# JasonTStanley/MultiDroneSim

Hardware: AMD Instinct MI355X
Metric: drone-steps/sec (whole node) at N_envs×N_drones; achieved HBM GB/s vs roofline (higher is better)
Workload: dtype f32

## Files before the change

include/mds.h:

```cpp
#ifndef MDS_H
#define MDS_H

#include <stddef.h>
#include <stdint.h>

#ifdef __cplusplus
extern "C" {
#endif

#define MDS_VERSION 202
#define MDS_OBS_DIM 20
#define MDS_ACT_DIM 4
#define MDS_STATE_DIM 13
#define MDS_DES_DIM 11
#define MDS_LEM_DIM 7
#define MDS_GEO_AUX_DIM 13

typedef enum mds_status {
  MDS_OK = 0,
  MDS_EINVAL = -1,
  MDS_ENOMEM = -2,
  MDS_EHIP = -3,
  MDS_EALIGN = -4,
  MDS_ESTATE = -5,
// ... 55 lines not shown
int mds_step(mds_handle* h, const void* action_dev, void* obs_dev, void* stream);

int mds_set_wind(mds_handle* h, const double force_world[3]);

#define MDS_SEG_DIM 40
int mds_set_trajectory_segments(mds_handle* h, const double* segs_host, const int32_t* offsets_host,
                                const int32_t* compound_host, const double* anchor_host, int32_t total_segments, void* stream);
int mds_traj_eval(mds_handle* h, double t, void* des_dev, void* stream);

int mds_set_lemniscate(mds_handle* h, const double* params_host, void* stream);
int mds_traj_yaw_free(mds_handle* h);
int mds_set_traj_specialisation(mds_handle* h, int on);
int mds_traj_phase_periodic(mds_handle* h);
int mds_set_traj_phase_table(mds_handle* h, int on);
int mds_get_last_rollout_phase_table(mds_handle* h);
int mds_set_geometric_gains(mds_handle* h, const mds_geometric_gains* gains);

int mds_step_geometric(mds_handle* h, double t, void* obs_dev, void* action_dev, void* stream);

int mds_rollout_geometric(mds_handle* h, double t0, int n_steps, void* obs_dev, int obs_every_step, void* stream);

int mds_rollout_step(mds_handle* h, const void* actions_dev, int n_action_sets, int first_step, int n_steps, void* obs_log_dev,
                     int log_slots, int episode_len, void* stream);
int mds_rollout_step_fused(mds_handle* h, const void* actions_dev, int n_action_sets, int first_step, int n_steps, void* obs_log_dev,
                           int log_slots, int episode_len, int steps_per_launch, void* stream);
int mds_reset_async(mds_handle* h, void* stream);

typedef struct mds_episode_params {
  int32_t max_steps;
  int32_t reserved;
// ... 155 lines not shown
```

multidronesim_amd/_capi.py:

```python
from __future__ import annotations

import ctypes as C
import os

_HERE = os.path.dirname(os.path.abspath(__file__))
LIB_PATH = os.environ.get("MDS_LIB_PATH") or os.path.join(_HERE, "libmds.so")

MDS_OK = 0
MDS_F32, MDS_F64, MDS_F16, MDS_F32C = 0, 1, 2, 3
MDS_PHYSICS_DYN, MDS_PHYSICS_DYN_DRAG, MDS_PHYSICS_DYN_GND, MDS_PHYSICS_DYN_DW, MDS_PHYSICS_DYN_GND_DRAG_DW = 0, 1, 2, 3, 4
MDS_INTEGRATOR_EULER, MDS_INTEGRATOR_RK4 = 0, 1
MDS_CF2X, MDS_CF2P = 0, 1
OBS_DIM, ACT_DIM, STATE_DIM, DES_DIM, LEM_DIM, GEO_AUX_DIM, SEG_DIM = 20, 4, 13, 11, 7, 13, 40


class MdsConfig(C.Structure):
    _fields_ = [("num_envs", C.c_int32), ("num_drones", C.c_int32), ("dtype", C.c_int32), ("physics", C.c_int32),
                ("integrator", C.c_int32), ("drone_model", C.c_int32), ("pyb_freq", C.c_int32),
                ("ctrl_freq", C.c_int32), ("device", C.c_int32), ("track_last_rpm", C.c_int32),
                ("M", C.c_double), ("L", C.c_double), ("KF", C.c_double), ("KM", C.c_double), ("J", C.c_double * 3),
                ("G", C.c_double), ("thrust2weight", C.c_double), ("drag_coeff", C.c_double * 3)]


class MdsGeometricGains(C.Structure):
# ... 47 lines not shown
    "mds_get_derived": (C.c_int, [_P, _PD]),
    "mds_reset": (C.c_int, [_P, _PD, _PD, _P]),
    "mds_state_ptrs": (C.c_int, [_P, C.POINTER(C.c_void_p), C.POINTER(C.c_size_t), C.POINTER(C.c_void_p)]),
    "mds_get_state": (C.c_int, [_P, _PD, _P]),
    "mds_set_state": (C.c_int, [_P, _PD, _P]),
    "mds_set_origin": (C.c_int, [_P, _PD, _P]),
    "mds_get_obs": (C.c_int, [_P, _P, _P]),
    "mds_step": (C.c_int, [_P, _P, _P, _P]),
    "mds_set_wind": (C.c_int, [_P, _PD]),
    "mds_set_lemniscate": (C.c_int, [_P, _PD, _P]),
    "mds_traj_yaw_free": (C.c_int, [_P]),
    "mds_set_traj_specialisation": (C.c_int, [_P, C.c_int]),
    "mds_traj_phase_periodic": (C.c_int, [_P]),
    "mds_set_traj_phase_table": (C.c_int, [_P, C.c_int]),
    "mds_get_last_rollout_phase_table": (C.c_int, [_P]),
    "mds_set_trajectory_segments": (C.c_int, [_P, _PD, C.POINTER(C.c_int32), C.POINTER(C.c_int32), _PD, C.c_int32, _P]),
    "mds_traj_eval": (C.c_int, [_P, C.c_double, _P, _P]),
    "mds_set_geometric_gains": (C.c_int, [_P, C.POINTER(MdsGeometricGains)]),
    "mds_step_geometric": (C.c_int, [_P, C.c_double, _P, _P, _P]),
    "mds_rollout_geometric": (C.c_int, [_P, C.c_double, C.c_int, _P, C.c_int, _P]),
    "mds_set_rollout_streams": (C.c_int, [_P, C.c_int]),
    "mds_get_last_rollout_streams": (C.c_int, [_P]),
    "mds_rollout_streams_for": (C.c_int, [_P, C.c_int, C.c_int]),
    "mds_set_rollout_form": (C.c_int, [_P, C.c_int, C.c_int]),
    "mds_rollout_form_for": (C.c_int, [_P, C.c_int]),
    "mds_get_last_rollout_form": (C.c_int, [_P]),
    "mds_rollout_step": (C.c_int, [_P, _P, C.c_int, C.c_int, C.c_int, _P, C.c_int, C.c_int, _P]),
    "mds_rollout_step_fused": (C.c_int, [_P, _P, C.c_int, C.c_int, C.c_int, _P, C.c_int, C.c_int, C.c_int, _P]),
    "mds_reset_async": (C.c_int, [_P, _P]),
    "mds_default_episode_params": (C.c_int, [C.POINTER(MdsEpisodeParams)]),
# ... 120 lines not shown
```

multidronesim_amd/csrc/mds_api.hip:

```cpp
#include <hip/hip_runtime.h>
#include <math.h>
#include <stdio.h>
#include <stdlib.h>
#include <string.h>

#include <new>
#include <type_traits>
#include <unordered_map>
#include <vector>

#include "../../include/mds.h"
#include "mds_consts.hpp"
#include "mds_devmem.hpp"
#include "mds_kernels.hip"
#include "mds_traj_image.hpp"
#ifndef MDS_PART
#define MDS_PART 3
#endif
#if MDS_PART & 1
#include "mds_episode_kernels.hip"
#endif
#if MDS_PART & 2
#include "mds_cbf_kernels.hip"
#include "mds_fedce_kernels.hip"
// ... 99 lines not shown
  void* lem = nullptr;
  double* scratch = nullptr;
  double* init_pose = nullptr;
  bool has_traj = false;
  int traj_mode = 0;
  bool traj_yaw_free = false;
  bool traj_spec = true;
  bool traj_phase_periodic = false;
  bool phase_tab_on = true;
  void* phase_tab = nullptr;
  bool phase_tab_filled = false;
  int phase_tab_rows = 0;
  int phase_tab_row = 0;
  double phase_tab_t = 0.0;
  int last_rollout_phase_table = 0;
  double* segs = nullptr;
  int nseg_total = 0;
  int* tinfo = nullptr;
  HostParams<float> p32 = {};
  HostParams<double> p64 = {};
  bool has_cbf = false;
  mds_cbf_params cbf = {};
  int* pair_ij = nullptr;
  void* obstacles = nullptr;
  int* cbf_order = nullptr;
  int* cbf_count = nullptr;
  int cbf_calls_half[2] = {-1, -1};
  int* cbf_cost = nullptr;
  int cbf_calls = -1;
  int rollout_streams = 0;
// ... 626 lines not shown
  return envfx_return_home(h, home, st);
}

int mds_step(mds_handle* h, const void* action, void* obs, void* stream) {
  MDS_DEV(h);
  if (!h || !action) return fail(MDS_EINVAL, "mds_step: null argument");
  if (!aligned16(action) || !aligned16(obs)) return fail(MDS_EALIGN, "mds_step: action_dev/obs_dev");
  if (int rc = step_plain(h, action, obs, Chain{(hipStream_t)stream, 0, 0})) return rc;
  return check_launches();
}

constexpr int kPhaseTabRows = 2048;
static bool phase_table_built(const mds_handle* h) {
  return h->cfg.dtype == MDS_F32 && h->cfg.integrator != MDS_INTEGRATOR_RK4 && !has_drag(h) && !h->envfx;
}
static size_t phase_table_bytes(const mds_handle* h) { return (size_t)kPhaseTabRows * kPhaseLanes * 2 * comp_size(h->cfg.dtype); }

int mds_set_lemniscate(mds_handle* h, const double* params, void* stream) {
  MDS_DEV(h);
  if (!h || !params) return fail(MDS_EINVAL, "mds_set_lemniscate: null argument");
  hipStream_t st = (hipStream_t)stream;
  const int n = h->n;
  double* centres = new (std::nothrow) double[(size_t)n * 3];
  if (!centres) return fail(MDS_ENOMEM, "mds_set_lemniscate: host allocation");
  bool yaw_free = true;
  for (int i = 0; i < n; ++i) {
    for (int k = 0; k < 3; ++k) centres[(size_t)3 * i + k] = params[(size_t)7 * i + 2 + k];
    yaw_free = yaw_free && params[(size_t)7 * i + 5] == 0.0;
  }
  const bool phase_periodic = lemniscate_phase_periodic(params, n);
  if (yaw_free && phase_periodic && phase_table_built(h))
    if (int arc = h->mem.alloc(&h->phase_tab, phase_table_bytes(h))) {
      delete[] centres;
      return arc;
    }
  int rc = mds_set_origin(h, centres, stream);
  delete[] centres;
  if (rc != MDS_OK) return rc;
  MDS_HIP(hipMemcpyAsync(h->scratch, params, (size_t)n * 7 * sizeof(double), hipMemcpyHostToDevice, st));
  with_dtype(h->cfg.dtype, [&](auto DT) {
    using T = typename decltype(DT)::T;
    k_set_planes<T><<<grid_for(n, 256), 256, 0, st>>>(n, h->ld, 7, h->scratch, (T*)h->lem);
  });
  MDS_HIP(hipGetLastError());
  MDS_HIP(hipStreamSynchronize(st));
  h->has_traj = true;
  h->traj_mode = 1;
  h->traj_yaw_free = yaw_free;
  h->traj_phase_periodic = phase_periodic;
  h->phase_tab_filled = false;
  return MDS_OK;
}

int mds_traj_yaw_free(mds_handle* h) { return h && h->traj_yaw_free ? 1 : 0; }
int mds_traj_phase_periodic(mds_handle* h) { return h && h->traj_phase_periodic ? 1 : 0; }

int mds_set_traj_specialisation(mds_handle* h, int on) {
  if (!h) return fail(MDS_EINVAL, "mds_set_traj_specialisation: null handle");
  h->traj_spec = on != 0;
  return MDS_OK;
}

int mds_set_traj_phase_table(mds_handle* h, int on) {
  if (!h) return fail(MDS_EINVAL, "mds_set_traj_phase_table: null handle");
  h->phase_tab_on = on != 0;
  return MDS_OK;
}

int mds_get_last_rollout_phase_table(mds_handle* h) { return h ? h->last_rollout_phase_table : 0; }

static bool use_yaw_free(const mds_handle* h) { return h->traj_mode == 1 && h->traj_yaw_free && h->traj_spec; }

int mds_set_trajectory_segments(mds_handle* h, const double* segs, const int32_t* offsets, const int32_t* compound,
                                const double* anchor, int32_t total, void* stream) {
  MDS_DEV(h);
  if (!h || !segs || !offsets || !compound || !anchor) return fail(MDS_EINVAL, "mds_set_trajectory_segments: null argument");
  const int n = h->n;
  std::vector<int> ti;
  std::vector<double> fm;
  int nu = 0;
  const char* why = "";
  const int brc = build_traj_image(segs, offsets, compound, n, total, fm, ti, nu, &why);
  if (brc != MDS_OK) return fail(brc, why);
  if (int rc = h->mem.alloc(&h->tinfo, sizeof(int) * 3 * n)) return rc;
  const int rc = h->mem.replace(&h->segs, sizeof(double) * fm.size(), [&](void* new_segs) -> int {
    MDS_HIP(hipMemcpy(new_segs, fm.data(), sizeof(double) * fm.size(), hipMemcpyHostToDevice));
    if (int orc = mds_set_origin(h, anchor, stream)) return orc;
    MDS_HIP(hipMemcpy(h->tinfo, ti.data(), sizeof(int) * 3 * n, hipMemcpyHostToDevice));
    return MDS_OK;
  });
  if (rc != MDS_OK) return rc;
  h->nseg_total = nu;
  h->has_traj = true;
  h->traj_mode = 2;
  h->traj_yaw_free = false;
  h->traj_phase_periodic = false;
  return MDS_OK;
}

int mds_traj_eval(mds_handle* h, double t, void* des, void* stream) {
  MDS_DEV(h);
  if (!h || !des) return fail(MDS_EINVAL, "mds_traj_eval: null argument");
  if (h->traj_mode == 1) return mds_lemniscate_eval(h, t, des, stream);
  if (h->traj_mode != 2) return fail(MDS_ESTATE, "mds_traj_eval: no trajectories set");
  hipStream_t st = (hipStream_t)stream;
  with_dtype(h->cfg.dtype, [&](auto DT) {
    using S = typename decltype(DT)::S;
    k_traj_eval<S><<<grid_for(h->n, 256), 256, 0, st>>>(h->n, t, SegTable{h->segs, h->nseg_total}, h->tinfo, (S*)des);
  });
  MDS_HIP(hipGetLastError());
  return MDS_OK;
// ... 42 lines not shown
                                   (S*)h->state_lo);
    });
  }, use_yaw_free(h), obs != nullptr, act != nullptr, rk4, drag);
  return MDS_OK;
}

int mds_step_geometric(mds_handle* h, double t, void* obs, void* act, void* stream) {
  MDS_DEV(h);
  if (!h) return fail(MDS_EINVAL, "mds_step_geometric: null handle");
  if (!h->has_traj) return fail(MDS_ESTATE, "mds_step_geometric: call mds_set_lemniscate first");
  if (!aligned16(obs) || !aligned16(act)) return fail(MDS_EALIGN, "mds_step_geometric: obs_dev/action_dev");
  if (int rc = step_geometric(h, t, obs, act, Chain{(hipStream_t)stream, 0, 0})) return rc;
  return check_launches();
}

static const float* phase_table_rows(mds_handle* h, double t0, double dt, int n_steps, hipStream_t st) {
  using T = float;
  const bool continues = h->phase_tab_filled && memcmp(&t0, &h->phase_tab_t, sizeof(double)) == 0;
  if (!continues || h->phase_tab_row + n_steps > h->phase_tab_rows) {
    const int rows = continues ? std::min(kPhaseTabRows, std::max(2 * h->phase_tab_rows, n_steps)) : n_steps;
    k_lemniscate_phase_table<T><<<grid_for((size_t)rows * kPhaseLanes, 256), 256, 0, st>>>(h->n, h->ld, t0, dt, rows, (const T*)h->lem, (T*)h->phase_tab);
    h->phase_tab_filled = true;
    h->phase_tab_rows = rows;
    h->phase_tab_row = 0;
  }
  const T* first = (const T*)h->phase_tab + (size_t)h->phase_tab_row * kPhaseLanes * 2;
  h->phase_tab_row += n_steps;
  for (int k = 0; k < n_steps; ++k) t0 += dt;
  h->phase_tab_t = t0;
  return first;
}
static bool use_phase_table(const mds_handle* h, int n_steps, hipStream_t st) {
  return use_yaw_free(h) && h->traj_phase_periodic && h->phase_tab_on && h->phase_tab && n_steps >= 1 && n_steps <= kPhaseTabRows &&
         !stream_is_capturing(st);
}

static void launch_rollout_kernel(mds_handle* h, int ctrl, double t0, int n_steps, void* obs_log, size_t log_stride, void* obs_last, hipStream_t st) {
  const dim3 grid = grid_for(h->n, kBlock);
  const double dt = 1.0 / h->cfg.ctrl_freq;
  const int omode = obs_log == nullptr ? kObsLast : log_stride == 0 ? kObsInPlace : kObsLog;
  h->last_rollout_phase_table = 0;
  auto launch = [&](auto DT, auto CTRL) {
    using T = typename decltype(DT)::T; using S = typename decltype(DT)::S;
    constexpr int COMP = DT.COMP ? 1 : 0;
    const void* gain = nullptr;
    if constexpr (CTRL() >= 1) gain = h->gain_dev[CTRL() - 1];
    with_flags([&](auto RK4, auto DRAG) {
      auto roll = [&](auto OBS) {
        if (h->traj_mode == 2) {
          if constexpr (CTRL() <= 1)
            k_rollout_traj<T, S, RK4(), DRAG(), CTRL(), COMP, OBS()><<<grid, kBlock, 0, st>>>(
                params<T>(h).c, gain, h->n, h->ld, t0, dt, n_steps, (S*)h->state, (const T*)h->origin, SegTable{h->segs, h->nseg_total}, h->tinfo,
                (T*)rpm_track(h), (S*)obs_log, log_stride, (S*)obs_last, (S*)h->state_lo);
        } else {
          auto* k = &k_rollout_geometric<T, S, RK4(), DRAG(), CTRL(), COMP, OBS()>;
          if constexpr (CTRL() == 0 && std::is_same_v<S, float> && !RK4() && !DRAG() && COMP == 0 && OBS() >= 0)
            if (use_phase_table(h, n_steps, st)) {
              const T* rows = (const T*)phase_table_rows(h, t0, dt, n_steps, st);
              k_rollout_geometric_y0p<T, S, false, false, 0, OBS()><<<grid, kBlock, 0, st>>>(
                  params<T>(h).c, gain, h->n, h->ld, t0, dt, n_steps, (S*)h->state, (const T*)h->lem, (T*)rpm_track(h), (S*)obs_log, log_stride,
                  (S*)obs_last, (T*)h->ll, (const S*)obs_last, (S*)h->state_lo, rows);
              h->last_rollout_phase_table = 1;
              return;
            }
          if constexpr (CTRL() == 0)
            if (use_yaw_free(h)) k = &k_rollout_geometric_y0<T, S, RK4(), DRAG(), COMP, OBS()>;
          k<<<grid, kBlock, 0, st>>>(params<T>(h).c, gain, h->n, h->ld, t0, dt, n_steps, (S*)h->state, (const T*)h->lem, (T*)rpm_track(h), (S*)obs_log,
                                     log_stride, (S*)obs_last, (T*)h->ll, (const S*)obs_last, (S*)h->state_lo);
        }
      };
      constexpr bool kPerObs = sizeof(T) == 4 && !RK4() && !DRAG() && CTRL() == 0;
      if constexpr (kPerObs) with_int<kObsInPlace, kObsLog, kObsLast>(omode, roll);
      else roll(std::integral_constant<int, -1>{});
    }, h->cfg.integrator == MDS_INTEGRATOR_RK4, has_drag(h));
  };
  if (ctrl >= 2) with_int<2, 3>(ctrl, [&](auto CTRL) { with_dtype_no_half(h->cfg.dtype, [&](auto DT) { launch(DT, CTRL); }); });
  else with_int<1, 0>(ctrl, [&](auto CTRL) { with_dtype(h->cfg.dtype, [&](auto DT) { launch(DT, CTRL); }); });
// ... 1727 lines not shown
```

multidronesim_amd/csrc/mds_kernels.hip:

```cpp
#include <hip/hip_runtime.h>
#include <type_traits>

#include "mds_math.hpp"
#include "mds_traj.hpp"

namespace mds {

typedef _Float16 half_t;

constexpr int kBlock = 256;
constexpr int kWave = 64;
constexpr int kStepMinWaves = 4;

#if defined(__HIP_DEVICE_COMPILE__)
#define MDS_KEEP_V(x) asm volatile("" : "+v"(x))
#define MDS_KEEP_S(x) asm volatile("" : "+s"(x))
#else
#define MDS_KEEP_V(x) ((void)0)
#define MDS_KEEP_S(x) ((void)0)
#endif
#if defined(__HIP_DEVICE_COMPILE__) || defined(__HIPCC__)
#define MDS_CONST_AS __attribute__((address_space(4)))
#else
#define MDS_CONST_AS
// ... 622 lines not shown
  const int i = blockIdx.x * blockDim.x + threadIdx.x;
  if (i >= n) return;
  double d11[11];
  traj_eval(segs, traj_info(tinfo, i), t, d11);
  for (int k = 0; k < 11; ++k) des[(size_t)i * 11 + k] = (S)d11[k];
}

constexpr int kObsLast = 0, kObsInPlace = 1, kObsLog = 2;
template <typename T, bool RK4, bool DRAG, int CTRL, int COMP, int OBS> constexpr int rollout_min_waves() {
  return !(sizeof(T) == 4 && !RK4 && !DRAG && CTRL == 0 && COMP == 0) ? 1 : (OBS == kObsInPlace || OBS == kObsLog) ? 6 : OBS == kObsLast ? 5 : 1;
}
template <typename T> struct alignas(2 * sizeof(T)) PhaseSC {
  T s, c;
};
constexpr int kPhaseLanes = kWave;
template <typename T, typename S, bool RK4, bool DRAG, int CTRL, int COMP, int OBS, bool Y0, bool TAB = false>
__device__ __forceinline__ void rollout_geometric_body(
    unsigned char* lds, const Consts<T>& c_arg, const void* __restrict__ Kp, const int n, const size_t ld, double t, const double ctrl_dt,
    const int n_steps, S* __restrict__ state, const T* __restrict__ lem, T* __restrict__ last_rpm, S* __restrict__ obs_log,
    const size_t log_stride, S* __restrict__ obs_last, T* __restrict__ ll, const S* __restrict__ obs_prev, S* __restrict__ state_lo,
    const T* __restrict__ phase_tab = nullptr) {
  static_assert(!Y0 || CTRL == 0, "the yaw-free form is GeometricControl's");
  static_assert(!TAB || Y0, "the phase table serves the yaw-free form");
  const bool comp = COMP < 0 ? state_lo != nullptr : COMP != 0;
  const int omode = OBS < 0 ? (obs_log == nullptr ? kObsLast : log_stride == 0 ? kObsInPlace : kObsLog) : OBS;
  constexpr bool kLean = !RK4 && COMP != 1;
  const int i = blockIdx.x * kBlock + threadIdx.x;
  const bool valid = i < n;
  if (n <= 0) return;
  const size_t il = (size_t)min(i, n - 1);
  GeoIn<T> in;
  resid_zero(in.r);
  if (comp) load_resid<S, T>(state_lo, ld, il, in.r);
  T prev[4] = {T(0), T(0), T(0), T(0)};
  T thr[4] = {T(0), T(0), T(0), T(0)};
  LowLevelState<T> L;
  L.last_omega = L.integral = {T(0), T(0), T(0)};
  load_geo_in<T, S>(state, lem, ld, il, in);
// ... 3 lines not shown
    L = load_lowlevel(ll, ld, il);
    if (CTRL == 3) load4<S, T>(obs_prev + il * kObsDim + 16, thr);
  }
  constexpr bool kCarry = CTRL == 0 && OBS != kObsLast;
  Frame<T> F;
  if (kCarry) F = make_frame(in.s.q, in.s.w);
  ObsRowOffs row_offs = obs_row_offs<S, true>(i, threadIdx.x);
  ObsRowOffs* const ro = OBS != kObsLast ? &row_offs : nullptr;
  const unsigned tab_off = ((unsigned)il & (unsigned)(kPhaseLanes - 1)) * (unsigned)sizeof(PhaseSC<T>);
  const unsigned char* tab_row = reinterpret_cast<const unsigned char*>(phase_tab);
  auto tab_load = [&]() {
    unsigned off = tab_off;
    MDS_KEEP_V(off);
    return *reinterpret_cast<const PhaseSC<T>*>(tab_row + off);
  };
  PhaseSC<T> sc = {T(0), T(1)};
  if (TAB) {
    sc = tab_load();
    MDS_KEEP_V(sc.s);
    MDS_KEEP_V(sc.c);
    for (T* v : {&in.P.a, &in.P.omega, &in.P.cx, &in.P.cy, &in.P.cz, &in.s.p.x, &in.s.p.y, &in.s.p.z, &in.s.q[0], &in.s.q[1], &in.s.q[2], &in.s.q[3],
                 &in.s.v.x, &in.s.v.y, &in.s.v.z, &in.s.w.x, &in.s.w.y, &in.s.w.z})
      MDS_KEEP_V(*v);
  }
  for (int k = 0; k < n_steps; ++k) {
    T o[kObsDim];
    const bool last = k == n_steps - 1;
    const bool want = omode != kObsLast || (obs_last != nullptr && last);
#if defined(__HIP_DEVICE_COMPILE__)
    const Consts<T> MDS_CONST_AS* cp = (const Consts<T> MDS_CONST_AS*)__builtin_amdgcn_kernarg_segment_ptr();
    MDS_KEEP_S(cp);
    const Consts<T> c = kLean ? load_const(cp) : c_arg;
#else
    const Consts<T>& c = c_arg;
#endif
    T act[4], clipped[4];
    {
      if (kLean) {
        MDS_KEEP_V(in.P.a);
        if (!Y0) MDS_KEEP_V(in.P.yaw_rate);
      }
      const Desired<T> des = TAB ? lemniscate_from_sc<T, Y0>(in.P, sc.s, sc.c, t) : lemniscate_local<T, Y0>(in.P, t);
      if (TAB) {
        tab_row += last ? 0 : kPhaseLanes * sizeof(PhaseSC<T>);
        sc = tab_load();
      }
      T u[4];
      if (CTRL == 0) {
        if (!kCarry) {
          F = make_frame(in.s.q, in.s.w);
        } else if (kLean) {
          MDS_KEEP_V(F.r22m1);
          F.R.m[8] = T(1) + F.r22m1;
        }
        geometric_control<T, Y0>(c, in.s.p - des.p, F.R, in.s.v, F.av, des, u, nullptr);
      } else if (CTRL == 1) {
        lqr12_control<T>(c, *static_cast<const Lqr12Gain<T>*>(Kp), euler_from_quat(in.s.q), quat_rotate(in.s.q, in.s.w), in.s.v, in.s.p - des.p,
                         des.v, des.yaw, des.yaw_rate, u);
      } else if (CTRL == 2) {
        lqr_omega_control<T>(c, *static_cast<const LqrGain<T>*>(Kp), euler_from_quat(in.s.q), in.s.v, in.s.p, des.p, des.v, des.yaw, u);
      } else {
        lqr_yank_omega_control<T>(c, *static_cast<const LqrYoGain<T>*>(Kp), euler_from_quat(in.s.q), thr, in.s.v, in.s.p, des.p, des.v,
                                  des.yaw, u);
      }
      if (CTRL <= 1) input_to_action(c, u, act);
      else if (CTRL == 2) thrust_omega_control(c, (T)ctrl_dt, u, in.s.w, L, act);
      else yank_omega_control(c, (T)ctrl_dt, u, thr, in.s.w, L, act);
    }
    if (comp) aviary_step_comp<T, RK4, DRAG>(c, in.s, in.r, act, prev, clipped);
    else if (CTRL == 0) aviary_step<T, RK4, DRAG>(c, in.s, F, act, prev, clipped);
    else aviary_step<T, RK4, DRAG>(c, in.s, act, prev, clipped);
    if (CTRL == 3)
      for (int j = 0; j < 4; ++j) thr[j] = clipped[j];
    if (kCarry) {
      F = make_frame(in.s.q, in.s.w);
      if (want) pack_obs(in.s, F, V3<T>{in.P.cx, in.P.cy, in.P.cz}, clipped, o);
    } else if (want) {
      pack_obs(in.s, V3<T>{in.P.cx, in.P.cy, in.P.cz}, clipped, o);
    }
    if (TAB) {
      MDS_KEEP_V(sc.s);
      MDS_KEEP_V(sc.c);
    }
    if (valid && last && (DRAG || last_rpm)) {
      unsigned iu = (unsigned)i;
      MDS_KEEP_V(iu);
      for (int j = 0; j < 4; ++j) *lane_ptr(last_rpm + j * ld, iu) = DRAG ? prev[j] : clipped[j];
    }
    if (omode == kObsInPlace) write_obs_rows<S, T, true, kLean>(lds, obs_log, n, i, valid, o, ro);
    else if (omode == kObsLog) write_obs_rows<S, T, false, kLean>(lds, obs_log + (size_t)k * log_stride, n, i, valid, o, ro);
    if (omode != kObsInPlace && obs_last != nullptr && last) write_obs_rows<S, T, false, kLean>(lds, obs_last, n, i, valid, o, ro);
    if (!TAB) t = uniform_f64(t + ctrl_dt);
  }
  if (valid) {
    store_state<S, T>(state, ld, i, in.s);
// ... 16 lines not shown
__global__ __launch_bounds__(kBlock, (rollout_min_waves<T, RK4, DRAG, 0, COMP, OBS>())) void k_rollout_geometric_y0(
    const Consts<T> c_arg, const void* __restrict__ Kp, const int n, const size_t ld, double t, const double ctrl_dt, const int n_steps,
    S* __restrict__ state, const T* __restrict__ lem, T* __restrict__ last_rpm, S* __restrict__ obs_log, const size_t log_stride,
    S* __restrict__ obs_last, T* __restrict__ ll = nullptr, const S* __restrict__ obs_prev = nullptr, S* __restrict__ state_lo = nullptr) {
  __shared__ __align__(16) unsigned char lds[kBlock * kObsDim * sizeof(S)];
  rollout_geometric_body<T, S, RK4, DRAG, 0, COMP, OBS, true>(lds, c_arg, Kp, n, ld, t, ctrl_dt, n_steps, state, lem, last_rpm, obs_log,
                                                              log_stride, obs_last, ll, obs_prev, state_lo);
}

template <typename T, typename S, bool RK4, bool DRAG, int COMP = -1, int OBS = -1>
__global__ __launch_bounds__(kBlock, (rollout_min_waves<T, RK4, DRAG, 0, COMP, OBS>())) void k_rollout_geometric_y0p(
    const Consts<T> c_arg, const void* __restrict__ Kp, const int n, const size_t ld, double t, const double ctrl_dt, const int n_steps,
    S* __restrict__ state, const T* __restrict__ lem, T* __restrict__ last_rpm, S* __restrict__ obs_log, const size_t log_stride,
    S* __restrict__ obs_last, T* __restrict__ ll, const S* __restrict__ obs_prev, S* __restrict__ state_lo, const T* __restrict__ phase_tab) {
  __shared__ __align__(16) unsigned char lds[kBlock * kObsDim * sizeof(S)];
  rollout_geometric_body<T, S, RK4, DRAG, 0, COMP, OBS, true, true>(lds, c_arg, Kp, n, ld, t, ctrl_dt, n_steps, state, lem, last_rpm, obs_log,
                                                                    log_stride, obs_last, ll, obs_prev, state_lo, phase_tab);
}

template <typename T>
__global__ __launch_bounds__(256) void k_lemniscate_phase_table(const int n, const size_t ld, const double t0, const double ctrl_dt,
                                                                const int n_rows, const T* __restrict__ lem, T* __restrict__ phase_tab) {
  const int e = blockIdx.x * 256 + threadIdx.x, k = e / kPhaseLanes, l = e % kPhaseLanes;
  if (n <= 0 || k >= n_rows) return;
  const size_t i = (size_t)min(l, n - 1);
  const T omega = lem[4 * i + 1], phase_shift = lem[4 * i + 3];
  double t = t0;
#pragma unroll 8
  for (int j = 0; j < k; ++j) t = t + ctrl_dt;
  PhaseSC<T> sc;
  m_sincos(reduced_phase<T>(t, omega, phase_shift), &sc.s, &sc.c);
  reinterpret_cast<PhaseSC<T>*>(phase_tab)[e] = sc;
}

template <typename T, typename S, bool RK4, bool DRAG, int CTRL, int COMP = -1, int OBS = -1>
__global__ __launch_bounds__(kBlock) void k_rollout_traj(const Consts<T> c, const void* __restrict__ Kp, const int n, const size_t ld, double t,
                                                         const double ctrl_dt, const int n_steps, S* __restrict__ state,
                                                         const T* __restrict__ origin, const SegTable segs,
                                                         const int* __restrict__ tinfo, T* __restrict__ last_rpm,
                                                         S* __restrict__ obs_log, const size_t log_stride, S* __restrict__ obs_last,
                                                         S* __restrict__ state_lo = nullptr) {
  __shared__ __align__(16) unsigned char lds[kBlock * kObsDim * sizeof(S)];
  const bool comp = COMP < 0 ? state_lo != nullptr : COMP != 0;
  const int omode = OBS < 0 ? (obs_log == nullptr ? kObsLast : log_stride == 0 ? kObsInPlace : kObsLog) : OBS;
  const int i = blockIdx.x * kBlock + threadIdx.x;
  const bool valid = i < n;
  State<T> s;
// ... 585 lines not shown
```

multidronesim_amd/csrc/mds_math.hpp:

```cpp
#pragma once
#include <math.h>
#include <stdint.h>

#if defined(__HIPCC__)
#define MDS_HD __host__ __device__ __forceinline__
#else
#define MDS_HD inline
#endif

namespace mds {

#if defined(__HIP_DEVICE_COMPILE__)
MDS_HD float m_rcp(float x) { return __builtin_amdgcn_rcpf(x); }
MDS_HD float m_sqrt(float x) { return __builtin_amdgcn_sqrtf(x); }
MDS_HD float m_rsqrt(float x) { return __builtin_amdgcn_rsqf(x); }
#else
MDS_HD float m_rcp(float x) { return 1.0f / x; }
MDS_HD float m_sqrt(float x) { return sqrtf(x); }
MDS_HD float m_rsqrt(float x) { return 1.0f / sqrtf(x); }
#endif
MDS_HD double m_rcp(double x) { return 1.0 / x; }
MDS_HD double m_sqrt(double x) { return sqrt(x); }
MDS_HD double m_rsqrt(double x) { return 1.0 / sqrt(x); }
MDS_HD float m_fma(float a, float b, float c) { return fmaf(a, b, c); }
MDS_HD double m_fma(double a, double b, double c) { return fma(a, b, c); }
template <typename T> MDS_HD T m_mul_rn(T a, T b) {
  T r = a * b;
#if defined(__HIP_DEVICE_COMPILE__)
  asm("" : "+v"(r));
#else
  asm("" : "+m"(r));
#endif
  return r;
}
MDS_HD float m_rint(float x) { return rintf(x); }
MDS_HD double m_rint(double x) { return rint(x); }
MDS_HD float m_exp(float x) { return expf(x); }
MDS_HD double m_exp(double x) { return exp(x); }
MDS_HD float m_abs(float x) { return fabsf(x); }
MDS_HD double m_abs(double x) { return fabs(x); }
// ... 625 lines not shown
  T sy = T(0), cy = T(1);
  if (P.yaw_rate != T(0)) {
    const T ph = reduced_phase<T>(t, P.yaw_rate, T(0));
    m_sincos(ph, &sy, &cy);
  }
  d.yaw = T(3.14159265358979323846) * sy;
  d.yaw_rate = T(3.14159265358979323846) * P.yaw_rate * cy;
  return d;
}
template <typename T, bool Y0 = false> MDS_HD Desired<T> lemniscate_local(const LemniscateParams<T>& P, double t) {
  T s, c;
  m_sincos(reduced_phase<T>(t, P.omega, P.phase_shift), &s, &c);
  return lemniscate_from_sc<T, Y0>(P, s, c, t);
}

inline bool lemniscate_phase_periodic(const double* params, long n) {
  for (long i = 64; i < n; ++i)
    if (params[7 * i + 1] != params[7 * (i - 64) + 1] || params[7 * i + 6] != params[7 * (i - 64) + 6]) return false;
  return true;
}

template <typename T> MDS_HD void input_to_action(const Consts<T>& c, const T u_in[4], T rpm[4]) {
  const T u0 = m_max(u_in[0], T(0));
  const T a = T(0.25) * u0, b1 = u_in[1] * c.inv_2L, b2 = u_in[2] * c.inv_2L, d = u_in[3] * c.inv_4r;
  T th[4] = {a - b2 - d, a + b1 + d, a + b2 - d, a - b1 + d};
  for (int i = 0; i < 4; ++i) {
    th[i] = m_clamp(th[i], c.min_motor_thrust, c.max_motor_thrust);
    rpm[i] = m_sqrt(th[i] * c.inv_kf);
  }
}
template <typename T> MDS_HD void action_to_input(const Consts<T>& c, const T action[4], int cap_rpm, T u[4]) {
  T r[4];
  for (int i = 0; i < 4; ++i) r[i] = cap_rpm ? m_clamp(action[i], T(0), c.max_rpm) : action[i];
  u[0] = c.kf * ((r[0] * r[0] + r[1] * r[1]) + (r[2] * r[2] + r[3] * r[3]));
  u[1] = c.arm_kf * ((r[1] - r[3]) * (r[1] + r[3]));
  u[2] = c.arm_kf * ((r[2] - r[0]) * (r[2] + r[0]));
  u[3] = c.km * ((r[1] - r[0]) * (r[1] + r[0]) + (r[3] - r[2]) * (r[3] + r[2]));
}

template <typename T> struct GeoAux {
  T force;
  V3<T> w_des;
  V3<T> b1d, b2d, b3d;
};
template <typename T, bool Y0 = false>
MDS_HD void geometric_control(const Consts<T>& c, V3<T> p_rel, const M3<T>& R, V3<T> v_world, V3<T> w,
                              const Desired<T>& des, T u[4], GeoAux<T>* aux) {
  const V3<T> Kp = {c.kp[0], c.kp[1], c.kp[2]}, Kv = {c.kv[0], c.kv[1], c.kv[2]};
  const V3<T> v_b = mulT(R, v_world);
  V3<T> RTvd, tw;
  if (Y0) {
    RTvd = {m_fma(R.m[0], des.v.x, R.m[3] * des.v.y), m_fma(R.m[1], des.v.x, R.m[4] * des.v.y), m_fma(R.m[2], des.v.x, R.m[5] * des.v.y)};
  } else {
    RTvd = mulT(R, des.v);
  }
  const V3<T> ev = v_b - RTvd;
  if (Y0) {
    tw = {des.a.x - Kp.x * p_rel.x, des.a.y - Kp.y * p_rel.y, c.g_ctrl - m_mul_rn(Kp.z, p_rel.z)};
  } else {
    tw = des.a - hadamard(Kp, p_rel);
    tw.z += c.g_ctrl;
  }
  const V3<T> fb_m = mulT(R, tw) - hadamard(Kv, ev) - cross(w, RTvd);
  V3<T> f_w = mul(R, c.mass * fb_m);
  T f2 = dot(f_w, f_w);
  T inv_fn = m_rsqrt(f2);
  if (f_w.z * inv_fn < c.cos_max_tilt) {
    const T scale = f_w.z * c.tan_max_tilt * m_rsqrt(m_fma(f_w.x, f_w.x, f_w.y * f_w.y));
    f_w.x *= scale;
    f_w.y *= scale;
    f2 = dot(f_w, f_w);
    inv_fn = m_rsqrt(f2);
// ... 330 lines not shown
```

multidronesim_amd/envs/BaseAviary.py:

```python
from __future__ import annotations

import ctypes as C
import time

import numpy as np
import torch

from .. import _capi as capi
from .._device import DTYPE_BY_NAME, TORCH_DTYPE, default_device_index, forget_env_device, note_env_device, require_gpu, stream_ptr, to_device
from ..utils.enums import DroneModel, Physics

__all__ = ["BaseAviary", "DroneModel", "Physics"]

_PHYSICS_MAP = {Physics.DYN: capi.MDS_PHYSICS_DYN, Physics.PYB: capi.MDS_PHYSICS_DYN,
                Physics.PYB_DRAG: capi.MDS_PHYSICS_DYN_DRAG, Physics.PYB_GND: capi.MDS_PHYSICS_DYN_GND,
                Physics.PYB_DW: capi.MDS_PHYSICS_DYN_DW, Physics.PYB_GND_DRAG_DW: capi.MDS_PHYSICS_DYN_GND_DRAG_DW}
_MODEL_MAP = {DroneModel.CF2X: capi.MDS_CF2X, DroneModel.CF2P: capi.MDS_CF2P}
_PYB_SUBSTITUTED = (Physics.PYB, Physics.PYB_DRAG, Physics.PYB_GND, Physics.PYB_DW, Physics.PYB_GND_DRAG_DW)
_CONSTANT_KEYS = {"M": 1, "L": 1, "KF": 1, "KM": 1, "J": 3, "G": 1, "thrust2weight": 1, "drag_coeff": 3}


def apply_constants(cfg, constants):
    for key, val in (constants or {}).items():
        if key not in _CONSTANT_KEYS:
# ... 461 lines not shown
        self._require_open()
        capi.check(self._lib.mds_set_traj_specialisation(self._h, C.c_int(1 if on else 0)), "mds_set_traj_specialisation")

    def traj_phase_periodic(self) -> bool:
        self._require_open()
        return bool(self._lib.mds_traj_phase_periodic(self._h))

    def set_traj_phase_table(self, on: bool = True):
        self._require_open()
        capi.check(self._lib.mds_set_traj_phase_table(self._h, C.c_int(1 if on else 0)), "mds_set_traj_phase_table")

    def last_rollout_phase_table(self) -> bool:
        self._require_open()
        return bool(self._lib.mds_get_last_rollout_phase_table(self._h))

    def rollout_form_for(self, n_steps: int) -> int:
        self._require_open()
        return int(self._lib.mds_rollout_form_for(self._h, C.c_int(int(n_steps))))

    def last_rollout_form(self) -> int:
        self._require_open()
        return int(self._lib.mds_get_last_rollout_form(self._h))

    def rollout_geometric_fused(self, t0: float, n_steps: int, log: bool = False, log_out: torch.Tensor | None = None,
                                controller: str = "geometric"):
        self._require_open()
        if log and log_out is None:
            log_out = torch.empty((n_steps, self.NUM_ENVS, self.NUM_DRONES, capi.OBS_DIM), dtype=self.dtype, device=self.device)
        fn = {"lqr": self._lib.mds_rollout_lqr_fused, "geometric": self._lib.mds_rollout_geometric_fused,
              "nominal": self._lib.mds_rollout_nominal_fused}[controller]
# ... 139 lines not shown
```

Before: 83.61 billion.

## Precompute per-lane lemniscate desired-state terms into a widened phase table

Extends the per-step phase table (sin/cos per lane) to an eight-value desired-state table holding the lemniscate position, velocity and acceleration terms, used when the amplitude is also 64-lane periodic. A new rollout kernel variant reads two float4 rows per step and skips the per-drone lemniscate evaluation inside the geometric controller, replacing arithmetic with cached table loads. The cost is a table four times larger to fill and read each step, plus extra live vector registers for the prefetched rows.

```diff
diff --git a/include/mds.h b/include/mds.h
--- a/include/mds.h
+++ b/include/mds.h
@@ -93,6 +93,9 @@
 int mds_traj_phase_periodic(mds_handle* h);
 int mds_set_traj_phase_table(mds_handle* h, int on);
 int mds_get_last_rollout_phase_table(mds_handle* h);
+int mds_traj_desired_periodic(mds_handle* h);
+int mds_set_traj_desired_table(mds_handle* h, int on);
+int mds_get_last_rollout_desired_table(mds_handle* h);
 int mds_set_geometric_gains(mds_handle* h, const mds_geometric_gains* gains);
 
 int mds_step_geometric(mds_handle* h, double t, void* obs_dev, void* action_dev, void* stream);
diff --git a/multidronesim_amd/_capi.py b/multidronesim_amd/_capi.py
--- a/multidronesim_amd/_capi.py
+++ b/multidronesim_amd/_capi.py
@@ -85,6 +85,9 @@
     "mds_traj_phase_periodic": (C.c_int, [_P]),
     "mds_set_traj_phase_table": (C.c_int, [_P, C.c_int]),
     "mds_get_last_rollout_phase_table": (C.c_int, [_P]),
+    "mds_traj_desired_periodic": (C.c_int, [_P]),
+    "mds_set_traj_desired_table": (C.c_int, [_P, C.c_int]),
+    "mds_get_last_rollout_desired_table": (C.c_int, [_P]),
     "mds_set_trajectory_segments": (C.c_int, [_P, _PD, C.POINTER(C.c_int32), C.POINTER(C.c_int32), _PD, C.c_int32, _P]),
     "mds_traj_eval": (C.c_int, [_P, C.c_double, _P, _P]),
     "mds_set_geometric_gains": (C.c_int, [_P, C.POINTER(MdsGeometricGains)]),
diff --git a/multidronesim_amd/csrc/mds_api.hip b/multidronesim_amd/csrc/mds_api.hip
--- a/multidronesim_amd/csrc/mds_api.hip
+++ b/multidronesim_amd/csrc/mds_api.hip
@@ -137,6 +137,11 @@
   int phase_tab_row = 0;
   double phase_tab_t = 0.0;
   int last_rollout_phase_table = 0;
+  bool traj_desired_periodic = false;
+  bool desired_tab_on = true;
+  size_t phase_tab_bytes = 0;
+  bool phase_tab_wide = false;
+  int last_rollout_desired_table = 0;
   double* segs = nullptr;
   int nseg_total = 0;
   int* tinfo = nullptr;
@@ -793,7 +798,7 @@
 static bool phase_table_built(const mds_handle* h) {
   return h->cfg.dtype == MDS_F32 && h->cfg.integrator != MDS_INTEGRATOR_RK4 && !has_drag(h) && !h->envfx;
 }
-static size_t phase_table_bytes(const mds_handle* h) { return (size_t)kPhaseTabRows * kPhaseLanes * 2 * comp_size(h->cfg.dtype); }
+static size_t phase_table_bytes(const mds_handle* h, bool wide) { return (size_t)kPhaseTabRows * kPhaseLanes * (wide ? 8 : 2) * comp_size(h->cfg.dtype); }
 
 int mds_set_lemniscate(mds_handle* h, const double* params, void* stream) {
   MDS_DEV(h);
@@ -807,12 +812,19 @@
     for (int k = 0; k < 3; ++k) centres[(size_t)3 * i + k] = params[(size_t)7 * i + 2 + k];
     yaw_free = yaw_free && params[(size_t)7 * i + 5] == 0.0;
   }
-  const bool phase_periodic = lemniscate_phase_periodic(params, n);
-  if (yaw_free && phase_periodic && phase_table_built(h))
-    if (int arc = h->mem.alloc(&h->phase_tab, phase_table_bytes(h))) {
-      delete[] centres;
-      return arc;
+  const bool phase_periodic = lemniscate_phase_periodic(params, n), desired_periodic = lemniscate_desired_periodic(params, n);
+  if (yaw_free && phase_periodic && phase_table_built(h)) {
+    const size_t want = phase_table_bytes(h, desired_periodic);
+    if (h->phase_tab_bytes < want) {
+      const int arc = h->phase_tab ? h->mem.replace(&h->phase_tab, want, [](void*) { return 0; }) : h->mem.alloc(&h->phase_tab, want);
+      if (arc) {
+        delete[] centres;
+        return arc;
+      }
+      h->phase_tab_bytes = want;
+      h->phase_tab_filled = false;
     }
+  }
   int rc = mds_set_origin(h, centres, stream);
   delete[] centres;
   if (rc != MDS_OK) return rc;
@@ -827,12 +839,14 @@
   h->traj_mode = 1;
   h->traj_yaw_free = yaw_free;
   h->traj_phase_periodic = phase_periodic;
+  h->traj_desired_periodic = desired_periodic;
   h->phase_tab_filled = false;
   return MDS_OK;
 }
 
 int mds_traj_yaw_free(mds_handle* h) { return h && h->traj_yaw_free ? 1 : 0; }
 int mds_traj_phase_periodic(mds_handle* h) { return h && h->traj_phase_periodic ? 1 : 0; }
+int mds_traj_desired_periodic(mds_handle* h) { return h && h->traj_desired_periodic ? 1 : 0; }
 
 int mds_set_traj_specialisation(mds_handle* h, int on) {
   if (!h) return fail(MDS_EINVAL, "mds_set_traj_specialisation: null handle");
@@ -846,7 +860,14 @@
   return MDS_OK;
 }
 
+int mds_set_traj_desired_table(mds_handle* h, int on) {
+  if (!h) return fail(MDS_EINVAL, "mds_set_traj_desired_table: null handle");
+  h->desired_tab_on = on != 0;
+  return MDS_OK;
+}
+
 int mds_get_last_rollout_phase_table(mds_handle* h) { return h ? h->last_rollout_phase_table : 0; }
+int mds_get_last_rollout_desired_table(mds_handle* h) { return h ? h->last_rollout_desired_table : 0; }
 
 static bool use_yaw_free(const mds_handle* h) { return h->traj_mode == 1 && h->traj_yaw_free && h->traj_spec; }
 
@@ -874,6 +895,7 @@
   h->traj_mode = 2;
   h->traj_yaw_free = false;
   h->traj_phase_periodic = false;
+  h->traj_desired_periodic = false;
   return MDS_OK;
 }
 
@@ -946,17 +968,19 @@
   return check_launches();
 }
 
-static const float* phase_table_rows(mds_handle* h, double t0, double dt, int n_steps, hipStream_t st) {
+static const float* phase_table_rows(mds_handle* h, double t0, double dt, int n_steps, bool wide, hipStream_t st) {
   using T = float;
-  const bool continues = h->phase_tab_filled && memcmp(&t0, &h->phase_tab_t, sizeof(double)) == 0;
+  const bool continues = h->phase_tab_filled && h->phase_tab_wide == wide && memcmp(&t0, &h->phase_tab_t, sizeof(double)) == 0;
   if (!continues || h->phase_tab_row + n_steps > h->phase_tab_rows) {
     const int rows = continues ? std::min(kPhaseTabRows, std::max(2 * h->phase_tab_rows, n_steps)) : n_steps;
-    k_lemniscate_phase_table<T><<<grid_for((size_t)rows * kPhaseLanes, 256), 256, 0, st>>>(h->n, h->ld, t0, dt, rows, (const T*)h->lem, (T*)h->phase_tab);
+    auto* const fill = wide ? &k_lemniscate_phase_table<T, true> : &k_lemniscate_phase_table<T, false>;
+    fill<<<grid_for((size_t)rows * kPhaseLanes, 256), 256, 0, st>>>(h->n, h->ld, t0, dt, rows, (const T*)h->lem, (T*)h->phase_tab);
     h->phase_tab_filled = true;
+    h->phase_tab_wide = wide;
     h->phase_tab_rows = rows;
     h->phase_tab_row = 0;
   }
-  const T* first = (const T*)h->phase_tab + (size_t)h->phase_tab_row * kPhaseLanes * 2;
+  const T* first = (const T*)h->phase_tab + (size_t)h->phase_tab_row * kPhaseLanes * (wide ? 8 : 2);
   h->phase_tab_row += n_steps;
   for (int k = 0; k < n_steps; ++k) t0 += dt;
   h->phase_tab_t = t0;
@@ -966,12 +990,15 @@
   return use_yaw_free(h) && h->traj_phase_periodic && h->phase_tab_on && h->phase_tab && n_steps >= 1 && n_steps <= kPhaseTabRows &&
          !stream_is_capturing(st);
 }
+static bool use_desired_table(const mds_handle* h, int n_steps, hipStream_t st) {
+  return use_phase_table(h, n_steps, st) && h->traj_desired_periodic && h->desired_tab_on && h->phase_tab_bytes >= phase_table_bytes(h, true);
+}
 
 static void launch_rollout_kernel(mds_handle* h, int ctrl, double t0, int n_steps, void* obs_log, size_t log_stride, void* obs_last, hipStream_t st) {
   const dim3 grid = grid_for(h->n, kBlock);
   const double dt = 1.0 / h->cfg.ctrl_freq;
   const int omode = obs_log == nullptr ? kObsLast : log_stride == 0 ? kObsInPlace : kObsLog;
-  h->last_rollout_phase_table = 0;
+  h->last_rollout_phase_table = h->last_rollout_desired_table = 0;
   auto launch = [&](auto DT, auto CTRL) {
     using T = typename decltype(DT)::T; using S = typename decltype(DT)::S;
     constexpr int COMP = DT.COMP ? 1 : 0;
@@ -988,11 +1015,13 @@
           auto* k = &k_rollout_geometric<T, S, RK4(), DRAG(), CTRL(), COMP, OBS()>;
           if constexpr (CTRL() == 0 && std::is_same_v<S, float> && !RK4() && !DRAG() && COMP == 0 && OBS() >= 0)
             if (use_phase_table(h, n_steps, st)) {
-              const T* rows = (const T*)phase_table_rows(h, t0, dt, n_steps, st);
-              k_rollout_geometric_y0p<T, S, false, false, 0, OBS()><<<grid, kBlock, 0, st>>>(
-                  params<T>(h).c, gain, h->n, h->ld, t0, dt, n_steps, (S*)h->state, (const T*)h->lem, (T*)rpm_track(h), (S*)obs_log, log_stride,
-                  (S*)obs_last, (T*)h->ll, (const S*)obs_last, (S*)h->state_lo, rows);
+              const bool wide = use_desired_table(h, n_steps, st);
+              const T* rows = (const T*)phase_table_rows(h, t0, dt, n_steps, wide, st);
+              auto* const kt = wide ? &k_rollout_geometric_y0d<T, S, false, false, 0, OBS()> : &k_rollout_geometric_y0p<T, S, false, false, 0, OBS()>;
+              kt<<<grid, kBlock, 0, st>>>(params<T>(h).c, gain, h->n, h->ld, t0, dt, n_steps, (S*)h->state, (const T*)h->lem, (T*)rpm_track(h),
+                                          (S*)obs_log, log_stride, (S*)obs_last, (T*)h->ll, (const S*)obs_last, (S*)h->state_lo, rows);
               h->last_rollout_phase_table = 1;
+              h->last_rollout_desired_table = wide ? 1 : 0;
               return;
             }
           if constexpr (CTRL() == 0)
diff --git a/multidronesim_amd/csrc/mds_kernels.hip b/multidronesim_amd/csrc/mds_kernels.hip
--- a/multidronesim_amd/csrc/mds_kernels.hip
+++ b/multidronesim_amd/csrc/mds_kernels.hip
@@ -660,7 +660,8 @@
   T s, c;
 };
 constexpr int kPhaseLanes = kWave;
-template <typename T, typename S, bool RK4, bool DRAG, int CTRL, int COMP, int OBS, bool Y0, bool TAB = false>
+constexpr int kTabNone = 0, kTabPhase = 1, kTabDesired = 2;
+template <typename T, typename S, bool RK4, bool DRAG, int CTRL, int COMP, int OBS, bool Y0, int TAB = kTabNone>
 __device__ __forceinline__ void rollout_geometric_body(
     unsigned char* lds, const Consts<T>& c_arg, const void* __restrict__ Kp, const int n, const size_t ld, double t, const double ctrl_dt,
     const int n_steps, S* __restrict__ state, const T* __restrict__ lem, T* __restrict__ last_rpm, S* __restrict__ obs_log,
@@ -668,6 +669,7 @@
     const T* __restrict__ phase_tab = nullptr) {
   static_assert(!Y0 || CTRL == 0, "the yaw-free form is GeometricControl's");
   static_assert(!TAB || Y0, "the phase table serves the yaw-free form");
+  static_assert(TAB != kTabDesired || (CTRL == 0 && sizeof(T) == 4), "the desired-state table serves the fp32 GeometricControl loop");
   const bool comp = COMP < 0 ? state_lo != nullptr : COMP != 0;
   const int omode = OBS < 0 ? (obs_log == nullptr ? kObsLast : log_stride == 0 ? kObsInPlace : kObsLog) : OBS;
   constexpr bool kLean = !RK4 && COMP != 1;
@@ -701,8 +703,28 @@
     MDS_KEEP_V(off);
     return *reinterpret_cast<const PhaseSC<T>*>(tab_row + off);
   };
+  const unsigned tab8_off = ((unsigned)il & (unsigned)(kPhaseLanes - 1)) * (unsigned)sizeof(Quad<T>);
+  typedef T Row4 __attribute__((vector_size(4 * sizeof(T))));
+  Row4 row_a = {}, row_b = {};
+  auto tab8_load = [&](unsigned off) {
+    row_a = *reinterpret_cast<const Row4*>(tab_row + off);
+    row_b = *reinterpret_cast<const Row4*>(tab_row + off + kPhaseLanes * sizeof(Quad<T>));
+  };
+  auto tab8_keep = [&]() {
+#if defined(__HIP_DEVICE_COMPILE__)
+    asm volatile("" : "+v"(row_a), "+v"(row_b));
+#endif
+  };
   PhaseSC<T> sc = {T(0), T(1)};
-  if (TAB) {
+  if (TAB == kTabDesired) {
+    unsigned off = tab8_off;
+    MDS_KEEP_V(off);
+    tab8_load(off);
+    tab8_keep();
+    for (T* v : {&in.P.cx, &in.P.cy, &in.P.cz, &in.s.p.x, &in.s.p.y, &in.s.p.z, &in.s.q[0], &in.s.q[1], &in.s.q[2], &in.s.q[3],
+                 &in.s.v.x, &in.s.v.y, &in.s.v.z, &in.s.w.x, &in.s.w.y, &in.s.w.z})
+      MDS_KEEP_V(*v);
+  } else if (TAB) {
     sc = tab_load();
     MDS_KEEP_V(sc.s);
     MDS_KEEP_V(sc.c);
@@ -723,6 +745,28 @@
 #endif
     T act[4], clipped[4];
     {
+      if constexpr (TAB == kTabDesired) {
+        if (kCarry) {
+          MDS_KEEP_V(F.r22m1);
+          F.R.m[8] = T(1) + F.r22m1;
+        } else {
+          F = make_frame(in.s.q, in.s.w);
+        }
+        const LemDesired8<T> d8 = {row_a[0], row_a[1], row_a[2], row_a[3], row_b[0], row_b[1], row_b[2], row_b[3]};
+        GeoPre<T> pre;
+        const V3<T> p_rel = desired8_p_rel(d8, in.s.p);
+        desired8_pre(d8, c.kp[0], c.kp[1], p_rel, F.R, pre);
+        tab_row += last ? 0 : kPhaseLanes * sizeof(LemDesired8<T>);
+        unsigned off = tab8_off;
+#if defined(__HIP_DEVICE_COMPILE__)
+        asm volatile("" : "+v"(off) : "v"(pre.RTvd.x), "v"(pre.RTvd.y), "v"(pre.RTvd.z), "v"(pre.tw_x), "v"(pre.tw_y), "v"(p_rel.x), "v"(p_rel.y));
+#endif
+        tab8_load(off);
+        Desired<T> des = {};
+        T u[4];
+        geometric_control<T, true, true>(c, p_rel, F.R, in.s.v, F.av, des, u, nullptr, &pre);
+        input_to_action(c, u, act);
+      } else {
       if (kLean) {
         MDS_KEEP_V(in.P.a);
         if (!Y0) MDS_KEEP_V(in.P.yaw_rate);
@@ -753,6 +797,7 @@
       if (CTRL <= 1) input_to_action(c, u, act);
       else if (CTRL == 2) thrust_omega_control(c, (T)ctrl_dt, u, in.s.w, L, act);
       else yank_omega_control(c, (T)ctrl_dt, u, thr, in.s.w, L, act);
+      }
     }
     if (comp) aviary_step_comp<T, RK4, DRAG>(c, in.s, in.r, act, prev, clipped);
     else if (CTRL == 0) aviary_step<T, RK4, DRAG>(c, in.s, F, act, prev, clipped);
@@ -765,7 +810,9 @@
     } else if (want) {
       pack_obs(in.s, V3<T>{in.P.cx, in.P.cy, in.P.cz}, clipped, o);
     }
-    if (TAB) {
+    if (TAB == kTabDesired) {
+      tab8_keep();
+    } else if (TAB) {
       MDS_KEEP_V(sc.s);
       MDS_KEEP_V(sc.c);
     }
@@ -812,23 +859,40 @@
     S* __restrict__ state, const T* __restrict__ lem, T* __restrict__ last_rpm, S* __restrict__ obs_log, const size_t log_stride,
     S* __restrict__ obs_last, T* __restrict__ ll, const S* __restrict__ obs_prev, S* __restrict__ state_lo, const T* __restrict__ phase_tab) {
   __shared__ __align__(16) unsigned char lds[kBlock * kObsDim * sizeof(S)];
-  rollout_geometric_body<T, S, RK4, DRAG, 0, COMP, OBS, true, true>(lds, c_arg, Kp, n, ld, t, ctrl_dt, n_steps, state, lem, last_rpm, obs_log,
-                                                                    log_stride, obs_last, ll, obs_prev, state_lo, phase_tab);
-}
-
-template <typename T>
+  rollout_geometric_body<T, S, RK4, DRAG, 0, COMP, OBS, true, kTabPhase>(lds, c_arg, Kp, n, ld, t, ctrl_dt, n_steps, state, lem, last_rpm,
+                                                                         obs_log, log_stride, obs_last, ll, obs_prev, state_lo, phase_tab);
+}
+template <typename T, typename S, bool RK4, bool DRAG, int COMP = -1, int OBS = -1>
+__global__ __launch_bounds__(kBlock, (rollout_min_waves<T, RK4, DRAG, 0, COMP, OBS>())) void k_rollout_geometric_y0d(
+    const Consts<T> c_arg, const void* __restrict__ Kp, const int n, const size_t ld, double t, const double ctrl_dt, const int n_steps,
+    S* __restrict__ state, const T* __restrict__ lem, T* __restrict__ last_rpm, S* __restrict__ obs_log, const size_t log_stride,
+    S* __restrict__ obs_last, T* __restrict__ ll, const S* __restrict__ obs_prev, S* __restrict__ state_lo, const T* __restrict__ desired_tab) {
+  __shared__ __align__(16) unsigned char lds[kBlock * kObsDim * sizeof(S)];
+  rollout_geometric_body<T, S, RK4, DRAG, 0, COMP, OBS, true, kTabDesired>(lds, c_arg, Kp, n, ld, t, ctrl_dt, n_steps, state, lem, last_rpm,
+                                                                           obs_log, log_stride, obs_last, ll, obs_prev, state_lo, desired_tab);
+}
+
+template <typename T, bool WIDE = false>
 __global__ __launch_bounds__(256) void k_lemniscate_phase_table(const int n, const size_t ld, const double t0, const double ctrl_dt,
                                                                 const int n_rows, const T* __restrict__ lem, T* __restrict__ phase_tab) {
   const int e = blockIdx.x * 256 + threadIdx.x, k = e / kPhaseLanes, l = e % kPhaseLanes;
   if (n <= 0 || k >= n_rows) return;
   const size_t i = (size_t)min(l, n - 1);
   const T omega = lem[4 * i + 1], phase_shift = lem[4 * i + 3];
-  double t = t0;
-#pragma unroll 8
-  for (int j = 0; j < k; ++j) t = t + ctrl_dt;
+  const double t = lemniscate_table_time(t0, ctrl_dt, k);
   PhaseSC<T> sc;
   m_sincos(reduced_phase<T>(t, omega, phase_shift), &sc.s, &sc.c);
-  reinterpret_cast<PhaseSC<T>*>(phase_tab)[e] = sc;
+  if constexpr (WIDE) {
+    LemniscateParams<T> P = {};
+    P.a = lem[4 * i];
+    P.omega = omega;
+    const LemDesired8<T> d = lemniscate_desired8(P, sc.s, sc.c);
+    Quad<T>* const row = reinterpret_cast<Quad<T>*>(phase_tab) + (size_t)k * (2 * kPhaseLanes);
+    row[l] = {{d.inv, d.mx, d.my, d.inv3}};
+    row[kPhaseLanes + l] = {{d.vx, d.vy, d.Xx, d.Xy}};
+  } else {
+    reinterpret_cast<PhaseSC<T>*>(phase_tab)[e] = sc;
+  }
 }
 
 template <typename T, typename S, bool RK4, bool DRAG, int CTRL, int COMP = -1, int OBS = -1>
diff --git a/multidronesim_amd/csrc/mds_math.hpp b/multidronesim_amd/csrc/mds_math.hpp
--- a/multidronesim_amd/csrc/mds_math.hpp
+++ b/multidronesim_amd/csrc/mds_math.hpp
@@ -22,8 +22,19 @@
 MDS_HD double m_rcp(double x) { return 1.0 / x; }
 MDS_HD double m_sqrt(double x) { return sqrt(x); }
 MDS_HD double m_rsqrt(double x) { return 1.0 / sqrt(x); }
+#if defined(MDS_HOST_UNFUSED_FMA) && !defined(__HIPCC__)
+MDS_HD float m_fma(float a, float b, float c) {
+  volatile float ab = a * b;
+  return ab + c;
+}
+MDS_HD double m_fma(double a, double b, double c) {
+  volatile double ab = a * b;
+  return ab + c;
+}
+#else
 MDS_HD float m_fma(float a, float b, float c) { return fmaf(a, b, c); }
 MDS_HD double m_fma(double a, double b, double c) { return fma(a, b, c); }
+#endif
 template <typename T> MDS_HD T m_mul_rn(T a, T b) {
   T r = a * b;
 #if defined(__HIP_DEVICE_COMPILE__)
@@ -679,10 +690,61 @@
   return lemniscate_from_sc<T, Y0>(P, s, c, t);
 }
 
+template <typename T> struct alignas(4 * sizeof(T)) Quad {
+  T v[4];
+};
+template <typename T> struct LemDesired8 {
+  T inv, mx, my, inv3;
+  T vx, vy, Xx, Xy;
+};
+template <typename T> MDS_HD LemDesired8<T> lemniscate_desired8(const LemniscateParams<T>& P, T s, T c) {
+  LemDesired8<T> d;
+  d.inv = m_rcp(m_fma(s, s, T(1)));
+  const T s2 = s * s, c2 = c * c;
+  const T poly = m_fma(c2, m_fma(s, s, T(-1)), m_fma(s2, s2, s2));
+  const T aw = P.a * P.omega, naw = -aw;
+  const T q = T(1) + m_fma(T(2), c2, s2);
+  const T inv2 = d.inv * d.inv;
+  d.vx = inv2 * (poly * naw);
+  d.vy = inv2 * (q * (s * naw));
+  const T sin2 = m_mul_rn(c, s + s);
+  const T cos2 = m_fma(c, c, -s2), cos4 = m_fma(-sin2, sin2 + sin2, T(1));
+  const T aw2 = aw * P.omega;
+  d.mx = c * (s * P.a);
+  d.my = c * P.a;
+  d.inv3 = T(-0.125) * (d.inv * inv2);
+  d.Xx = m_fma(cos2, T(3), T(7)) * (sin2 * (T(4) * aw2));
+  d.Xy = (m_fma(T(44), cos2, cos4) + T(-21)) * (c * aw2);
+  return d;
+}
+template <typename T> MDS_HD V3<T> desired8_p_rel(const LemDesired8<T>& d, V3<T> p) {
+  return {m_fma(-d.inv, d.mx, p.x), m_fma(-d.inv, d.my, p.y), p.z};
+}
+template <typename T> struct GeoPre {
+  V3<T> RTvd;
+  T tw_x, tw_y;
+};
+template <typename T> MDS_HD void desired8_pre(const LemDesired8<T>& d, T kp_x, T kp_y, V3<T> p_rel, const M3<T>& R, GeoPre<T>& pre) {
+  pre.RTvd = {m_fma(R.m[0], d.vx, R.m[3] * d.vy), m_fma(R.m[1], d.vx, R.m[4] * d.vy), m_fma(R.m[2], d.vx, R.m[5] * d.vy)};
+  pre.tw_x = m_fma(d.inv3, d.Xx, -(kp_x * p_rel.x));
+  pre.tw_y = m_fma(d.inv3, d.Xy, -(kp_y * p_rel.y));
+}
+
 inline bool lemniscate_phase_periodic(const double* params, long n) {
   for (long i = 64; i < n; ++i)
     if (params[7 * i + 1] != params[7 * (i - 64) + 1] || params[7 * i + 6] != params[7 * (i - 64) + 6]) return false;
   return true;
+}
+MDS_HD double lemniscate_table_time(double t0, double ctrl_dt, int k) {
+  double t = t0;
+#pragma unroll 8
+  for (int j = 0; j < k; ++j) t = t + ctrl_dt;
+  return t;
+}
+inline bool lemniscate_desired_periodic(const double* params, long n) {
+  for (long i = 64; i < n; ++i)
+    if (params[7 * i] != params[7 * (i - 64)]) return false;
+  return lemniscate_phase_periodic(params, n);
 }
 
 template <typename T> MDS_HD void input_to_action(const Consts<T>& c, const T u_in[4], T rpm[4]) {
@@ -708,19 +770,24 @@
   V3<T> w_des;
   V3<T> b1d, b2d, b3d;
 };
-template <typename T, bool Y0 = false>
+template <typename T, bool Y0 = false, bool PRE = false>
 MDS_HD void geometric_control(const Consts<T>& c, V3<T> p_rel, const M3<T>& R, V3<T> v_world, V3<T> w,
-                              const Desired<T>& des, T u[4], GeoAux<T>* aux) {
+                              const Desired<T>& des, T u[4], GeoAux<T>* aux, const GeoPre<T>* pre = nullptr) {
+  static_assert(!PRE || Y0, "the ready-made terms are the yaw-free form's");
   const V3<T> Kp = {c.kp[0], c.kp[1], c.kp[2]}, Kv = {c.kv[0], c.kv[1], c.kv[2]};
   const V3<T> v_b = mulT(R, v_world);
   V3<T> RTvd, tw;
-  if (Y0) {
+  if constexpr (PRE) {
+    RTvd = pre->RTvd;
+  } else if (Y0) {
     RTvd = {m_fma(R.m[0], des.v.x, R.m[3] * des.v.y), m_fma(R.m[1], des.v.x, R.m[4] * des.v.y), m_fma(R.m[2], des.v.x, R.m[5] * des.v.y)};
   } else {
     RTvd = mulT(R, des.v);
   }
   const V3<T> ev = v_b - RTvd;
-  if (Y0) {
+  if constexpr (PRE) {
+    tw = {pre->tw_x, pre->tw_y, c.g_ctrl - m_mul_rn(Kp.z, p_rel.z)};
+  } else if (Y0) {
     tw = {des.a.x - Kp.x * p_rel.x, des.a.y - Kp.y * p_rel.y, c.g_ctrl - m_mul_rn(Kp.z, p_rel.z)};
   } else {
     tw = des.a - hadamard(Kp, p_rel);
diff --git a/multidronesim_amd/envs/BaseAviary.py b/multidronesim_amd/envs/BaseAviary.py
--- a/multidronesim_amd/envs/BaseAviary.py
+++ b/multidronesim_amd/envs/BaseAviary.py
@@ -499,6 +499,18 @@
         self._require_open()
         return bool(self._lib.mds_get_last_rollout_phase_table(self._h))
 
+    def traj_desired_periodic(self) -> bool:
+        self._require_open()
+        return bool(self._lib.mds_traj_desired_periodic(self._h))
+
+    def set_traj_desired_table(self, on: bool = True):
+        self._require_open()
+        capi.check(self._lib.mds_set_traj_desired_table(self._h, C.c_int(1 if on else 0)), "mds_set_traj_desired_table")
+
+    def last_rollout_desired_table(self) -> bool:
+        self._require_open()
+        return bool(self._lib.mds_get_last_rollout_desired_table(self._h))
+
     def rollout_form_for(self, n_steps: int) -> int:
         self._require_open()
         return int(self._lib.mds_rollout_form_for(self._h, C.c_int(int(n_steps))))
```

After: 85.72 billion, median of 6. +2.5%, better.
